# qq456cvb/CPPF

Hardware: AMD Instinct MI355X
Metric: point-pairs/sec (PPF+MLP+vote+argmax), N=4096 K=128; 1/2/4/8 GPU (higher is better)
Workload: dtype f32; 1 GPU; c2: single object N=4096 K=128 (P=524288 pairs), bottle config, res 0.004, grid 26x76x26, num_rots 72 adaptive, fused PPF+MLP(MFMA f32)+decode of the  ... (full text: bench_full.json); parallelism=objects x1

## Files before the change

### cppf_amd/csrc/pair_mlp.hip

```cpp
#include <hip/hip_runtime.h>
#include <stdint.h>
#include <string.h>

#include "../../include/cppf.h"
#include "cppf_math.h"

using namespace cppf;

typedef float f32x4 __attribute__((ext_vector_type(4)));
typedef float f32x2 __attribute__((ext_vector_type(2)));
typedef float f32x4u __attribute__((ext_vector_type(4), aligned(4)));

#define CPPF_CHECK_LAUNCH()                         \
    do {                                            \
        hipError_t e__ = hipGetLastError();         \
        if (e__ != hipSuccess) return (int)e__;     \
    } while (0)

#include "pair_layout.h"

static bool is_std(int F, const int* dims, int n_res, int out_dim)
{
    return F == STD_F && n_res == 3 && dims[0] == 84 && dims[1] == 32 && dims[2] == 32 && dims[3] == 16 &&
           out_dim >= 1 && out_dim <= 16 * STD_NOB;
}

#define GEN_MAX_RES 8
#define GEN_MAX_DIM 128
static bool gen_ok(int F, const int* dims, int n_res, int out_dim)
{
    if (n_res < 0 || n_res > GEN_MAX_RES || F < 1 || out_dim < 1 || out_dim > 1024) return false;
    if (dims[0] != 2 * F + 4) return false;
    for (int i = 0; i <= n_res; ++i)
        if (dims[i] < 1 || dims[i] > GEN_MAX_DIM) return false;
    return true;
}
static size_t gen_floats(const int* dims, int n_res, int out_dim)
{
    size_t n = 0;
    for (int i = 0; i < n_res; ++i) {
        size_t K = dims[i], M = dims[i + 1];
        n += M * K + M + M * M + M;
        if (K != M) n += M * K + M;
    }
    n += (size_t)out_dim * dims[n_res] + out_dim;
    return n;
}

extern "C" size_t cppf_pair_mlp_packed_floats(int F, const int* dims, int n_res, int out_dim)
{
    if (!dims) return 0;
    if (is_std(F, dims, n_res, out_dim)) return STD_PACKED;
    if (gen_ok(F, dims, n_res, out_dim)) return gen_floats(dims, n_res, out_dim);
    return 0;
}

extern "C" int cppf_pair_mlp_pack(const float* params, const int64_t* offs, int F, const int* dims, int n_res,
                                  int out_dim, float* out)
{
    if (!params || !offs || !dims || !out) return CPPF_EINVAL;
    if (is_std(F, dims, n_res, out_dim)) {
        if (offs[4] < 0 || offs[10] >= 0 || offs[16] < 0) return CPPF_EINVAL;
        for (int i = 0; i < STD_PACKED; ++i) out[i] = std_pack_elem(i, params, offs, out_dim);
        return 0;
    }
    if (gen_ok(F, dims, n_res, out_dim)) {
        size_t n = 0;
        for (int i = 0; i < n_res; ++i) {
            size_t K = dims[i], M = dims[i + 1];
            const int64_t* o = offs + 6 * i;
            if ((K != M) != (o[4] >= 0)) return CPPF_EINVAL;
            memcpy(out + n, params + o[0], sizeof(float) * M * K); n += M * K;
            memcpy(out + n, params + o[1], sizeof(float) * M); n += M;
            memcpy(out + n, params + o[2], sizeof(float) * M * M); n += M * M;
            memcpy(out + n, params + o[3], sizeof(float) * M); n += M;
            if (K != M) {
                memcpy(out + n, params + o[4], sizeof(float) * M * K); n += M * K;
                memcpy(out + n, params + o[5], sizeof(float) * M); n += M;
            }
        }
        const int64_t* o = offs + 6 * n_res;
        memcpy(out + n, params + o[0], sizeof(float) * out_dim * dims[n_res]); n += (size_t)out_dim * dims[n_res];
        memcpy(out + n, params + o[1], sizeof(float) * out_dim);
        return 0;
    }
    return CPPF_EUNSUPPORTED;
}

struct PackOffs { int64_t o[20]; };
__global__ __launch_bounds__(256) void pair_pack_kernel(const float* __restrict__ params, PackOffs offs, int out_dim,
                                                        float* __restrict__ out)
{
    const int i = blockIdx.x * 256 + threadIdx.x;
    if (i < STD_PACKED) out[i] = std_pack_elem(i, params, offs.o, out_dim);
}
extern "C" int cppf_pair_mlp_pack_device(const float* params, const int64_t* offs, int F, const int* dims, int n_res,
                                         int out_dim, float* out, void* stream)
{
    if (!params || !offs || !dims || !out) return CPPF_EINVAL;
    if (!is_std(F, dims, n_res, out_dim)) return CPPF_EUNSUPPORTED;
    if (offs[4] < 0 || offs[10] >= 0 || offs[16] < 0) return CPPF_EINVAL;
    PackOffs po;
    for (int i = 0; i < 20; ++i) po.o[i] = offs[i];
    hipLaunchKernelGGL(pair_pack_kernel, dim3((STD_PACKED + 255) / 256), dim3(256), 0, (hipStream_t)stream, params, po,
                       out_dim, out);
    hipError_t e = hipGetLastError();
    return e == hipSuccess ? 0 : (int)e;
}

#define MLP_THREADS 1024
#define MLP_WAVES_PER_SIMD 4
#define PB 1

__device__ __forceinline__ f32x4 mfma4(float a, float b, f32x4 c)
{
    return __builtin_amdgcn_mfma_f32_16x16x4f32(a, b, c, 0, 0, 0);
}
__device__ __forceinline__ float relu1(float v) { return fmaxf(v, 0.f); }
__device__ __forceinline__ f32x4 relu4(f32x4 v)
{
    f32x4 r;
    r[0] = relu1(v[0]); r[1] = relu1(v[1]); r[2] = relu1(v[2]); r[3] = relu1(v[3]);
    return r;
}
__device__ __forceinline__ f32x4 ldb4(const float* p) { return *reinterpret_cast<const f32x4*>(p); }

__device__ __forceinline__ float ppf_component(const float* __restrict__ pc, const float* __restrict__ nrm, int a, int b,
                                               int g)
{
    const f3 pa = ld3(pc, a), pb = ld3(pc, b), na = ld3(nrm, a), nb = ld3(nrm, b);
    const f3 xy = sub3(pa, pb);
    const float d = sqrtf((xy.x * xy.x + xy.y * xy.y) + xy.z * xy.z);
    const float den = d + 1e-7f;
    const f3 u = {xy.x / den, xy.y / den, xy.z / den};
    const float p0 = (na.x * u.x + na.y * u.y) + na.z * u.z;
    const float p1 = (nb.x * u.x + nb.y * u.y) + nb.z * u.z;
    const float p2 = (na.x * nb.x + na.y * nb.y) + na.z * nb.z;
    return g == 0 ? p0 : (g == 1 ? p1 : (g == 2 ? p2 : d));
}

__device__ __forceinline__ unsigned xor16u(unsigned v, int lane)
{
    (void)lane;
    return (unsigned)__builtin_amdgcn_ds_swizzle((int)v, 0x401f);
}
__device__ __forceinline__ unsigned xor32u(unsigned v, int lane)
{
    return (unsigned)__builtin_amdgcn_ds_bpermute((lane ^ 32) << 2, (int)v);
}
__device__ __forceinline__ float xor16f(float v, int lane) { return __uint_as_float(xor16u(__float_as_uint(v), lane)); }
__device__ __forceinline__ float xor32f(float v, int lane) { return __uint_as_float(xor32u(__float_as_uint(v), lane)); }

template <int NL>
__device__ __forceinline__ bool sample_seg(const float (&v)[NL], float u, int g, int lane, int& bin)
{
    static_assert(NL == 8 || NL == 9, "the draw below searches 7 running sums + at most one more");
    float m = v[0];
#pragma unroll
    for (int k = 1; k < NL; ++k) m = fmaxf(m, v[k]);
    float mall = fmaxf(m, xor16f(m, lane));
    mall = fmaxf(mall, xor32f(mall, lane));
    const float c = -(mall * CPPF_LOG2E);
    float e[NL];
#pragma unroll
    for (int k = 0; k < NL; ++k) e[k] = det_exp2w(v[k], c);
    float b[NL];
    b[0] = e[0];
#pragma unroll
    for (int k = 1; k < NL; ++k) b[k] = b[k - 1] + e[k];
    const float T = b[NL - 1];
    const float Tp = xor16f(T, lane);
    const float half = T + Tp;
    const float oth = xor32f(half, lane);
    const float off = ((g & 2) ? oth : 0.f) + ((g & 1) ? Tp : 0.f);
    const float t = u * ((g & 2) ? oth + half : half + oth) - off;
    const bool c1 = b[3] > t;
    const bool c2 = (c1 ? b[1] : b[5]) > t;
    const float lo = c2 ? b[0] : b[2], hi = c2 ? b[4] : b[6];
    const bool c3 = (c1 ? lo : hi) > t;
    int kk = (c1 ? 0 : 4) + (c2 ? 0 : 2) + (c3 ? 0 : 1);
    if (NL == 9) kk = b[7] > t ? kk : 8;
    const unsigned long long hm = __ballot(b[NL - 1] > t);
    const unsigned h0 = (unsigned)hm & 0xffffu, h1 = (unsigned)(hm >> 16) & 0xffffu, h2 = (unsigned)(hm >> 32) & 0xffffu;
    const unsigned o1 = h1 & ~h0, o2 = h2 & ~(h0 | h1), o3 = ~(h0 | h1 | h2) & 0xffffu;
    const unsigned long long own = (unsigned long long)(h0 | (o1 << 16)) | ((unsigned long long)(o2 | (o3 << 16)) << 32);
    bool owner = __builtin_amdgcn_inverse_ballot_w64(own);
    bin = NL * g + kk;
    if (__any(u < 0.f)) {
        asm volatile("" ::: "memory");
        int ak = 64;
#pragma unroll
        for (int k = NL - 1; k >= 0; --k)
            if (v[k] == mall) ak = k;
        const int am = NL * g + ak;
        int best = min(am, (int)xor16u((unsigned)am, lane));
        best = min(best, (int)xor32u((unsigned)best, lane));
        if (u < 0.f) { bin = best; owner = am == best; }
    }
    return owner;
}

struct MlpArgs {
    const float* pc;
    const float* nrm;
    const float* feat;
    const void* idxs;
    const float* packed;
    const float* u_tr;
    const float* u_rot;
    const float* table;
    float* out;
    float* outputs;
    float* heads;
    int64_t P;
    int out_dim;
    int idx64;
    float vr0, vr1;
    const int32_t* sel;
    const int32_t* n_sel;
};

template <typename T>
__device__ __forceinline__ const T& at_off(const void* base, unsigned byte_off)
{
    return *reinterpret_cast<const T*>(static_cast<const char*>(base) + byte_off);
}
template <typename T>
__device__ __forceinline__ T& at_off(void* base, unsigned byte_off)
{
    return *reinterpret_cast<T*>(static_cast<char*>(base) + byte_off);
}
__device__ __forceinline__ f3 ld3o(const float* __restrict__ base, int i)
{
    const unsigned o = __umul24((unsigned)i, 12u);
    return {at_off<float>(base, o), at_off<float>(base + 1, o), at_off<float>(base + 2, o)};
}

template <bool SEL>
__device__ __forceinline__ unsigned pair_row(const MlpArgs& A, int slot, int Pn)
{
    const unsigned s = (unsigned)min(slot, Pn - 1);
    return SEL ? (unsigned)at_off<int>(A.sel, s * 4u) : s;
}

template <bool SEL>
__device__ __forceinline__ void load_pair_idx(const MlpArgs& A, int slot, int Pn, int& ia, int& ib)
{
    const unsigned p = pair_row<SEL>(A, slot, Pn);
    const unsigned o = p * (A.idx64 ? 16u : 8u);
    ia = at_off<int>(A.idxs, o);
    ib = at_off<int>(static_cast<const char*>(A.idxs) + (A.idx64 ? 8 : 4), o);
}

__device__ __forceinline__ float ppf_from(f3 pa, f3 pb, f3 na, f3 nb, int g)
{
    const f3 xy = sub3(pa, pb);
    const float d = sqrt_rn((xy.x * xy.x + xy.y * xy.y) + xy.z * xy.z);
    const float den = d + 1e-7f;
    const float rden = refined_rcp(den);
    const f3 u = {div_by(xy.x, den, rden), div_by(xy.y, den, rden), div_by(xy.z, den, rden)};
    const float p0 = (na.x * u.x + na.y * u.y) + na.z * u.z;
    const float p1 = (nb.x * u.x + nb.y * u.y) + nb.z * u.z;
    const float p2 = (na.x * nb.x + na.y * nb.y) + na.z * nb.z;
    (void)g;
    const bool g0 = __builtin_amdgcn_inverse_ballot_w64(0x000000000000ffffull), g1 = __builtin_amdgcn_inverse_ballot_w64(0x00000000ffff0000ull),
               g2 = __builtin_amdgcn_inverse_ballot_w64(0x0000ffff00000000ull);
    const float s23 = g2 ? p2 : d, s123 = g1 ? p1 : s23;
    return g0 ? p0 : s123;
}

#define PROJ_PPB 8
__device__ __forceinline__ void point_proj_body(const float* __restrict__ feat, const float* __restrict__ packed, float* __restrict__ T,
                                                int64_t N)
{
    __shared__ float f[PROJ_PPB][STD_F];
    const int half = threadIdx.x >> 7, r = threadIdx.x & 127;
    const int64_t n0 = (int64_t)blockIdx.x * PROJ_PPB;
    for (int i = threadIdx.x; i < PROJ_PPB * STD_F; i += 256) {
        const int64_t n = n0 + i / STD_F;
        f[i / STD_F][i % STD_F] = n < N ? feat[n * STD_F + i % STD_F] : 0.f;
    }
    __syncthreads();
    float acc[PROJ_PPB / 2];
    const float b = r < 64 ? packed[OFF_BPT + r] : 0.f;
#pragma unroll
    for (int q = 0; q < PROJ_PPB / 2; ++q) acc[q] = b;
#pragma unroll 8
    for (int k = 0; k < STD_F; ++k) {
        const float w = packed[OFF_WPT + k * PROJ_COLS + r];
#pragma unroll
        for (int q = 0; q < PROJ_PPB / 2; ++q) acc[q] = fmaf(w, f[half + 2 * q][k], acc[q]);
    }
#pragma unroll
    for (int q = 0; q < PROJ_PPB / 2; ++q) {
        const int64_t n = n0 + half + 2 * q;
        if (n < N) T[n * PROJ_COLS + r] = acc[q];
    }
}
__global__ __launch_bounds__(256) void point_proj_kernel(const float* __restrict__ feat, const float* __restrict__ packed,
                                                         float* __restrict__ T, int64_t N)
{
    point_proj_body(feat, packed, T, N);
}
struct ProjBatch { const float* feat[8]; const float* packed[8]; float* table[8]; int64_t N[8]; };
__global__ __launch_bounds__(256) void point_proj_batch_kernel(ProjBatch B)
{
    const int i = blockIdx.y;
    if ((int64_t)blockIdx.x * PROJ_PPB >= B.N[i]) return;
    point_proj_body(B.feat[i], B.packed[i], B.table[i], B.N[i]);
}

template <bool LOGITS, bool DECODE, bool HEADS, bool SEL>
__device__ __forceinline__ void pair_mlp_body(const MlpArgs& A, const int wg, const int n_wg)
{
    extern __shared__ __attribute__((aligned(16))) float W[];
    {
        const f32x4* src = reinterpret_cast<const f32x4*>(A.packed);
        f32x4* dst = reinterpret_cast<f32x4*>(W);
        for (int k = threadIdx.x; k < STD_LDS / 4; k += MLP_THREADS) {
            int from = k;
            if (DECODE && k >= OFF_WF / 4 && k < OFF_B0B / 4) from = OFF_WFD / 4 + (k - OFF_WF / 4);
            if (DECODE && k >= OFF_BF / 4) from = OFF_BFD / 4 + (k - OFF_BF / 4);
            dst[k] = src[from];
        }
    }
    float* lut = W + STD_LDS;
    int* tile_ctr = reinterpret_cast<int*>(W + STD_LDS + 112);
    if (threadIdx.x == 0) *tile_ctr = 0;
    if (DECODE && threadIdx.x < 100) {
        const int k = threadIdx.x;
        float v;
        if (k < 32) v = ((float)k / 31.0f * 2.0f) * A.vr0 - A.vr0;
        else if (k < 64) v = (float)(k - 32) / 31.0f * A.vr1;
        else v = (float)(k - 64) / 35.0f * (float)CPPF_PI;
        lut[k] = v;
    }
    __syncthreads();

    const int lane = threadIdx.x & 63;
    const int j = lane & 15, g = lane >> 4;
    __builtin_assume(g >= 0 && g < 4);
    int Pn = (int)A.P;
    if (SEL) Pn = min(max(*A.n_sel, 0), Pn);
    const int n_tiles = (Pn + 16 * PB - 1) / (16 * PB);
    const int per_wg = (n_tiles + n_wg - 1) / n_wg;
    const int wg_begin = wg * per_wg;
    const int wg_end = min(wg_begin + per_wg, n_tiles);
    auto claim = [&]() -> int {
        int v = 0;
        if (lane == 0) v = atomicAdd(tile_ctr, 1);
        return wg_begin + __builtin_amdgcn_readfirstlane(v);
    };
    int cur = claim();
    if (cur >= wg_end) return;
    int nxt = claim();

    f32x4 acc[PB][4];
    int ia1[PB], ib1[PB];
    {
        f32x4 ta[PB][4], tb[PB][4];
        float xp[PB];
        int ia[PB], ib[PB];
#pragma unroll
        for (int pb = 0; pb < PB; ++pb) load_pair_idx<SEL>(A, cur * (16 * PB) + pb * 16 + j, Pn, ia[pb], ib[pb]);
#pragma unroll
        for (int pb = 0; pb < PB; ++pb) {
            const unsigned oa = (unsigned)ia[pb] * (PROJ_COLS * 4u) + 16u * g, ob_ = (unsigned)ib[pb] * (PROJ_COLS * 4u) + 256u + 16u * g;
#pragma unroll
            for (int ob = 0; ob < 4; ++ob) { ta[pb][ob] = at_off<f32x4>(A.table, oa + 64u * ob); tb[pb][ob] = at_off<f32x4>(A.table, ob_ + 64u * ob); }
            xp[pb] = ppf_from(ld3o(A.pc, ia[pb]), ld3o(A.pc, ib[pb]), ld3o(A.nrm, ia[pb]), ld3o(A.nrm, ib[pb]), g);
        }
        const int nt = nxt < wg_end ? nxt : cur;
#pragma unroll
        for (int pb = 0; pb < PB; ++pb) load_pair_idx<SEL>(A, nt * (16 * PB) + pb * 16 + j, Pn, ia1[pb], ib1[pb]);
        const f32x4 w = ldb4(W + OFF_W0P + lane * 4);
#pragma unroll
        for (int ob = 0; ob < 4; ++ob)
#pragma unroll
            for (int pb = 0; pb < PB; ++pb) acc[pb][ob] = mfma4(w[ob], xp[pb], ta[pb][ob] + tb[pb][ob]);
    }

    for (;;) {
        const int tile = cur;
        asm volatile("" ::: "memory");
        int pair[PB];
#pragma unroll
        for (int pb = 0; pb < PB; ++pb) pair[pb] = tile * (16 * PB) + pb * 16 + j;
        unsigned row[PB];
#pragma unroll
        for (int pb = 0; pb < PB; ++pb) row[pb] = pair_row<SEL>(A, pair[pb], Pn);

        f3 npa[PB], npb[PB], nna[PB], nnb[PB];
#pragma unroll
        for (int pb = 0; pb < PB; ++pb) {
            npa[pb] = ld3o(A.pc, ia1[pb]); npb[pb] = ld3o(A.pc, ib1[pb]);
            nna[pb] = ld3o(A.nrm, ia1[pb]); nnb[pb] = ld3o(A.nrm, ib1[pb]);
        }
        f32x2 ut[PB], ur[PB];
        if (DECODE) {
#pragma unroll
            for (int pb = 0; pb < PB; ++pb) {
                const unsigned po = row[pb] * 8u;
                if (!SEL) ut[pb] = at_off<f32x2>(A.u_tr, po);
                if (HEADS) ur[pb] = at_off<f32x2>(A.u_rot, po);
            }
        }

        f32x4 y[PB][2];
        {
            f32x4 h[PB][2], a2[PB][2];
#pragma unroll
            for (int pb = 0; pb < PB; ++pb) { h[pb][0] = relu4(acc[pb][0]); h[pb][1] = relu4(acc[pb][1]); }
#pragma unroll
            for (int ob = 0; ob < 2; ++ob) {
                const f32x4 b = ldb4(W + OFF_B0B + 16 * ob + 4 * g);
#pragma unroll
                for (int pb = 0; pb < PB; ++pb) a2[pb][ob] = b;
            }
#pragma unroll
            for (int s = 0; s < 8; ++s) {
                const f32x2 w = *reinterpret_cast<const f32x2*>(W + OFF_W0B + (s * 64 + lane) * 2);
#pragma unroll
                for (int ob = 0; ob < 2; ++ob)
#pragma unroll
                    for (int pb = 0; pb < PB; ++pb) a2[pb][ob] = mfma4(w[ob], h[pb][s >> 2][s & 3], a2[pb][ob]);
            }
#pragma unroll
            for (int pb = 0; pb < PB; ++pb) { y[pb][0] = a2[pb][0] + acc[pb][2]; y[pb][1] = a2[pb][1] + acc[pb][3]; }
        }
        {
            f32x4 a1[PB][2], h[PB][2], a2[PB][2];
#pragma unroll
            for (int ob = 0; ob < 2; ++ob) {
                const f32x4 b1 = ldb4(W + OFF_B1A + 16 * ob + 4 * g), b2 = ldb4(W + OFF_B1B + 16 * ob + 4 * g);
#pragma unroll
                for (int pb = 0; pb < PB; ++pb) { a1[pb][ob] = b1; a2[pb][ob] = b2; }
            }
#pragma unroll
            for (int s = 0; s < 8; ++s) {
                const f32x2 w = *reinterpret_cast<const f32x2*>(W + OFF_W1A + (s * 64 + lane) * 2);
#pragma unroll
                for (int ob = 0; ob < 2; ++ob)
#pragma unroll
                    for (int pb = 0; pb < PB; ++pb) a1[pb][ob] = mfma4(w[ob], y[pb][s >> 2][s & 3], a1[pb][ob]);
            }
#pragma unroll
            for (int pb = 0; pb < PB; ++pb) { h[pb][0] = relu4(a1[pb][0]); h[pb][1] = relu4(a1[pb][1]); }
#pragma unroll
            for (int s = 0; s < 8; ++s) {
                const f32x2 w = *reinterpret_cast<const f32x2*>(W + OFF_W1B + (s * 64 + lane) * 2);
#pragma unroll
                for (int ob = 0; ob < 2; ++ob)
#pragma unroll
                    for (int pb = 0; pb < PB; ++pb) a2[pb][ob] = mfma4(w[ob], h[pb][s >> 2][s & 3], a2[pb][ob]);
            }
#pragma unroll
            for (int pb = 0; pb < PB; ++pb) { y[pb][0] = a2[pb][0] + y[pb][0]; y[pb][1] = a2[pb][1] + y[pb][1]; }
        }
        f32x4 ta[PB][4], tb[PB][4];
        float xp[PB];
#pragma unroll
        for (int pb = 0; pb < PB; ++pb) {
            xp[pb] = ppf_from(npa[pb], npb[pb], nna[pb], nnb[pb], g);
            const unsigned oa = (unsigned)ia1[pb] * (PROJ_COLS * 4u) + 16u * g, ob_ = (unsigned)ib1[pb] * (PROJ_COLS * 4u) + 256u + 16u * g;
#pragma unroll
            for (int ob = 0; ob < 4; ++ob) { ta[pb][ob] = at_off<f32x4>(A.table, oa + 64u * ob); tb[pb][ob] = at_off<f32x4>(A.table, ob_ + 64u * ob); }
        }
        const int nxt2 = claim();
        {
            const int nt = nxt2 < wg_end ? nxt2 : tile;
#pragma unroll
            for (int pb = 0; pb < PB; ++pb) load_pair_idx<SEL>(A, nt * (16 * PB) + pb * 16 + j, Pn, ia1[pb], ib1[pb]);
        }

        f32x4 z[PB];
        {
            f32x4 a1[PB][2], a2[PB];
            {
                const f32x4 b1 = ldb4(W + OFF_B2 + 4 * g), b0 = ldb4(W + OFF_B2 + 16 + 4 * g), b2 = ldb4(W + OFF_B2B + 4 * g);
#pragma unroll
                for (int pb = 0; pb < PB; ++pb) { a1[pb][0] = b1; a1[pb][1] = b0; a2[pb] = b2; }
            }
#pragma unroll
            for (int s = 0; s < 8; ++s) {
                const f32x2 w = *reinterpret_cast<const f32x2*>(W + OFF_W2 + (s * 64 + lane) * 2);
#pragma unroll
                for (int ob = 0; ob < 2; ++ob)
#pragma unroll
                    for (int pb = 0; pb < PB; ++pb) a1[pb][ob] = mfma4(w[ob], y[pb][s >> 2][s & 3], a1[pb][ob]);
            }
#pragma unroll
            for (int s = 0; s < 4; ++s) {
                const float w = W[OFF_W2B + s * 64 + lane];
#pragma unroll
                for (int pb = 0; pb < PB; ++pb) {
                    const f32x4 h = relu4(a1[pb][0]);
                    a2[pb] = mfma4(w, h[s], a2[pb]);
                }
            }
#pragma unroll
            for (int pb = 0; pb < PB; ++pb) z[pb] = a2[pb] + a1[pb][1];
        }
        {
            const f32x4 w = ldb4(W + OFF_W0P + lane * 4);
#pragma unroll
            for (int ob = 0; ob < 4; ++ob)
#pragma unroll
                for (int pb = 0; pb < PB; ++pb) acc[pb][ob] = mfma4(w[ob], xp[pb], ta[pb][ob] + tb[pb][ob]);
        }
#pragma unroll
        for (int pb = 0; pb < PB; ++pb) {
            constexpr int NOB_USED = (DECODE && !HEADS) ? 4 : STD_NOB;
            f32x4 L[STD_NOB];
#pragma unroll
            for (int ob = 0; ob < NOB_USED; ++ob) L[ob] = ldb4(W + OFF_BF + 16 * ob + 4 * g);
#pragma unroll
            for (int s = 0; s < 4; ++s) {
                const float* wp = W + OFF_WF + (s * 64 + lane) * STD_NOBP;
                const f32x4 w0 = ldb4(wp), w1 = ldb4(wp + 4), w2 = ldb4(wp + 8);
#pragma unroll
                for (int ob = 0; ob < NOB_USED; ++ob) {
                    const float w = ob < 4 ? w0[ob & 3] : (ob < 8 ? w1[ob & 3] : w2[ob & 3]);
                    L[ob] = mfma4(w, z[pb][s], L[ob]);
                }
            }
            const bool live = pair[pb] < Pn;
            if (!LOGITS && !DECODE) {
                float sacc = 0.f;
#pragma unroll
                for (int ob = 0; ob < STD_NOB; ++ob) sacc += (L[ob][0] + L[ob][1]) + (L[ob][2] + L[ob][3]);
                if (sacc == 1.2345e30f) A.outputs[0] = sacc;
            }
            if (LOGITS) {
                if (live) {
                    float* o = A.out + (int64_t)pair[pb] * A.out_dim + 4 * g;
#pragma unroll
                    for (int ob = 0; ob < STD_NOB; ++ob) {
                        const int c0 = 16 * ob + 4 * g;
                        if (c0 + 3 < A.out_dim) {
                            *reinterpret_cast<f32x4u*>(o + 16 * ob) = L[ob];
                        } else {
#pragma unroll
                            for (int r = 0; r < 3; ++r)
                                if (c0 + r < A.out_dim) o[16 * ob + r] = L[ob][r];
                        }
                    }
                }
            }
            if (DECODE) {
                int k;
                if (!SEL) {
                    {
                        const float v[8] = {L[0][0], L[0][1], L[0][2], L[0][3], L[1][0], L[1][1], L[1][2], L[1][3]};
                        if (sample_seg<8>(v, ut[pb][0], g, lane, k) && live) at_off<float>(A.outputs, row[pb] * 8u) = lut[k];
                    }
                    {
                        const float v[8] = {L[2][0], L[2][1], L[2][2], L[2][3], L[3][0], L[3][1], L[3][2], L[3][3]};
                        if (sample_seg<8>(v, ut[pb][1], g, lane, k) && live) at_off<float>(A.outputs, row[pb] * 8u + 4u) = lut[32 + k];
                    }
                }
                if (HEADS) {
                    const unsigned ho = row[pb] * 32u;
                    {
                        const float v[9] = {L[4][0], L[4][1], L[4][2], L[4][3], L[5][0], L[5][1], L[5][2], L[5][3], L[8][0]};
                        if (sample_seg<9>(v, ur[pb][0], g, lane, k) && live) at_off<float>(A.heads, ho) = lut[64 + k];
                    }
                    {
                        const float v[9] = {L[6][0], L[6][1], L[6][2], L[6][3], L[7][0], L[7][1], L[7][2], L[7][3], L[8][1]};
                        if (sample_seg<9>(v, ur[pb][1], g, lane, k) && live) at_off<float>(A.heads, ho + 4u) = lut[64 + k];
                    }
                    if (live && g < 2) { f32x2 w; w[0] = L[8][2]; w[1] = L[8][3]; at_off<f32x2>(A.heads, ho + 8u + 8u * g) = w; }
                    if (live && g == 2) { f32x2 w; w[0] = L[8][2]; w[1] = 0.f; at_off<f32x2>(A.heads, ho + 24u) = w; }
                }
            }
        }
        cur = nxt;
        nxt = nxt2;
        if (cur >= wg_end) break;
    }
}

template <bool LOGITS, bool DECODE, bool HEADS, bool SEL = false>
__global__ __launch_bounds__(MLP_THREADS, MLP_WAVES_PER_SIMD) void pair_mlp_kernel(MlpArgs A)
{
    pair_mlp_body<LOGITS, DECODE, HEADS, SEL>(A, (int)blockIdx.x, (int)gridDim.x);
}

#define MLP_BATCH_MAX 8
struct MlpBatch {
    MlpArgs item[MLP_BATCH_MAX];
    int wg_begin[MLP_BATCH_MAX + 1];
    int n;
    int per_xcd;
};
static_assert(sizeof(ProjBatch) <= 4096, "ProjBatch travels by value: kernel arguments are limited to 4 KB");
static_assert(sizeof(MlpBatch) <= 4096, "MlpBatch travels by value: kernel arguments are limited to 4 KB");
template <bool HEADS, bool SEL = false>
__global__ __launch_bounds__(MLP_THREADS, MLP_WAVES_PER_SIMD) void pair_mlp_batch_kernel(MlpBatch B)
{
    if (!SEL && B.per_xcd > 0) {
        const int x = (int)blockIdx.x & 7, r = (int)blockIdx.x >> 3;
        const int i = x / B.per_xcd;
        pair_mlp_body<false, true, HEADS, false>(B.item[i], r * B.per_xcd + x % B.per_xcd, ((int)gridDim.x >> 3) * B.per_xcd);
        return;
    }
    int i = 0;
    while (i + 1 < B.n && (int)blockIdx.x >= B.wg_begin[i + 1]) ++i;
    pair_mlp_body<false, true, HEADS, SEL>(B.item[i], (int)blockIdx.x - B.wg_begin[i], B.wg_begin[i + 1] - B.wg_begin[i]);
}

struct GenArgs {
    const float* pc;
    const float* nrm;
    const float* feat;
    const void* idxs;
    const float* packed;
    float* out;
    int64_t P;
    int F, n_res, out_dim, idx64;
    int dims[GEN_MAX_RES + 1];
};
#define GEN_THREADS 64
__global__ __launch_bounds__(GEN_THREADS) void pair_mlp_generic_kernel(GenArgs A)
{
    extern __shared__ __attribute__((aligned(16))) float S[];
    int maxd = 0;
    for (int i = 0; i <= A.n_res; ++i) maxd = max(maxd, A.dims[i]);
    float* X = S;
    float* H = S + maxd * GEN_THREADS;
    const int t = threadIdx.x;
    for (int64_t p = (int64_t)blockIdx.x * GEN_THREADS + t; p < (A.P + GEN_THREADS - 1) / GEN_THREADS * GEN_THREADS;
         p += (int64_t)gridDim.x * GEN_THREADS) {
        const bool live = p < A.P;
        const int64_t pc_ = live ? p : A.P - 1;
        int ia, ib;
        if (A.idx64) {
            const longlong2 v = reinterpret_cast<const longlong2*>(A.idxs)[pc_];
            ia = (int)v.x; ib = (int)v.y;
        } else {
            const int2 v = reinterpret_cast<const int2*>(A.idxs)[pc_];
            ia = v.x; ib = v.y;
        }
        const int F = A.F;
        for (int k = 0; k < F; ++k) {
            X[k * GEN_THREADS + t] = A.feat[(int64_t)ia * F + k];
            X[(F + k) * GEN_THREADS + t] = A.feat[(int64_t)ib * F + k];
        }
        for (int c = 0; c < 4; ++c) X[(2 * F + c) * GEN_THREADS + t] = ppf_component(A.pc, A.nrm, ia, ib, c);
        const float* w = A.packed;
        for (int l = 0; l < A.n_res; ++l) {
            const int K = A.dims[l], M = A.dims[l + 1];
            const float *w1 = w, *b1 = w1 + M * K, *w2 = b1 + M, *b2 = w2 + M * M;
            const float *w0 = b2 + M, *b0 = w0 + M * K;
            const bool has0 = K != M;
            for (int o = 0; o < M; ++o) {
                float acc = b1[o];
                for (int k = 0; k < K; ++k) acc = fmaf(w1[o * K + k], X[k * GEN_THREADS + t], acc);
                H[o * GEN_THREADS + t] = acc > 0.f ? acc : 0.f;
            }
            for (int o = 0; o < M; ++o) {
                float acc = b2[o];
                for (int k = 0; k < M; ++k) acc = fmaf(w2[o * M + k], H[k * GEN_THREADS + t], acc);
                float skip;
                if (has0) {
                    float a0 = b0[o];
                    for (int k = 0; k < K; ++k) a0 = fmaf(w0[o * K + k], X[k * GEN_THREADS + t], a0);
                    skip = a0;
                } else {
                    skip = X[o * GEN_THREADS + t];
                }
                S[(2 * maxd + o) * GEN_THREADS + t] = acc + skip;
            }
            for (int o = 0; o < M; ++o) X[o * GEN_THREADS + t] = S[(2 * maxd + o) * GEN_THREADS + t];
            w = has0 ? b0 + M : b2 + M;
        }
        const int K = A.dims[A.n_res];
        const float *wf = w, *bf = wf + A.out_dim * K;
        for (int o = 0; o < A.out_dim; ++o) {
            float acc = bf[o];
            for (int k = 0; k < K; ++k) acc = fmaf(wf[o * K + k], X[k * GEN_THREADS + t], acc);
            if (live) A.out[p * A.out_dim + o] = acc;
        }
    }
}

__device__ int sample_bin_mem(const float* __restrict__ l, int nb, float u, int col0)
{
    (void)col0;
    float m = l[0];
    int am = 0;
    for (int k = 1; k < nb; ++k)
        if (l[k] > m) { m = l[k]; am = k; }
    if (u < 0.f) return am;
    const int NL = (nb + 3) / 4;
    const float c = -(m * CPPF_LOG2E);
    float T[4];
    for (int g = 0; g < 4; ++g) {
        float acc = 0.f;
        for (int k = g * NL; k < (g + 1) * NL && k < nb; ++k) {
            const float ek = det_exp2w(l[k], c);
            acc = k == g * NL ? ek : acc + ek;
        }
        T[g] = acc;
    }
    const float s01 = T[0] + T[1], s23 = T[2] + T[3];
    const float tt = u * (s01 + s23);
    const float off[4] = {0.f, T[0], s01, s01 + T[2]};
    for (int g = 0; g < 4; ++g) {
        const float t = tt - off[g];
        float b = 0.f;
        for (int k = g * NL; k < (g + 1) * NL && k < nb; ++k) {
            const float ek = det_exp2w(l[k], c);
            b = k == g * NL ? ek : b + ek;
            if (b > t) return k;
        }
    }
    return nb - 1;
}


__global__ __launch_bounds__(256) void decode_center_kernel(const float* __restrict__ logits, int64_t P, int ld, int nb,
                                                            float vr0, float vr1, const float* __restrict__ u,
                                                            float* __restrict__ outputs)
{
    const int64_t i = (int64_t)blockIdx.x * 256 + threadIdx.x;
    if (i >= 2 * P) return;
    const int64_t p = i >> 1;
    const int h = (int)(i & 1);
    const int k = sample_bin_mem(logits + p * ld + h * nb, nb, u[i], h * nb);
    const float d = (float)(nb - 1);
    outputs[i] = h == 0 ? ((float)k / d * 2.0f) * vr0 - vr0 : (float)k / d * vr1;
}

__global__ __launch_bounds__(256) void decode_rot_kernel(const float* __restrict__ logits, int64_t P, int ld, int out_dim,
                                                         int tb, int rb, const float* __restrict__ u,
                                                         float* __restrict__ heads)
{
    const int64_t i = (int64_t)blockIdx.x * 256 + threadIdx.x;
    if (i >= 2 * P) return;
    const int64_t p = i >> 1;
    const int h = (int)(i & 1);
    const float* l = logits + p * ld;
    const int k = sample_bin_mem(l + 2 * tb + h * rb, rb, u[i], 2 * tb + h * rb);
    float* o = heads + 8 * p;
    o[h] = (float)k / (float)(rb - 1) * (float)CPPF_PI;
    if (h == 0) { o[2] = l[out_dim - 5]; o[3] = l[out_dim - 4]; o[4] = l[out_dim - 3]; }
    else { o[5] = l[out_dim - 2]; o[6] = l[out_dim - 1]; o[7] = 0.f; }
}

static int mlp_grid(int64_t P)
{
    const int64_t tiles = (P + 16 * PB - 1) / (16 * PB);
    int64_t nb = (tiles + MLP_THREADS / 64 - 1) / (MLP_THREADS / 64);
    const int64_t resident = 256 * (MLP_WAVES_PER_SIMD * 4 / (MLP_THREADS / 64));
    if (nb > resident) nb = resident;
    if (nb < 1) nb = 1;
    return (int)nb;
}

extern "C" size_t cppf_pair_mlp_workspace_bytes(int64_t N, int F, const int* dims, int n_res, int out_dim)
{
    if (!dims || N < 0) return 0;
    return is_std(F, dims, n_res, out_dim) ? (size_t)N * PROJ_COLS * sizeof(float) : 0;
}

template <bool LOGITS, bool DECODE, bool HEADS, bool SEL = false>
static int launch_std(MlpArgs& A, int64_t N, void* workspace, size_t workspace_bytes, hipStream_t st)
{
    if (N < 1) return CPPF_EINVAL;
    if (N >= (1ll << 23) || A.P >= (1ll << 27)) return CPPF_EUNSUPPORTED;
    if (!workspace || workspace_bytes < (size_t)N * PROJ_COLS * sizeof(float)) return CPPF_EWORKSPACE;
    float* table = static_cast<float*>(workspace);
    if (!SEL) {
        hipLaunchKernelGGL(point_proj_kernel, dim3((unsigned)((N + PROJ_PPB - 1) / PROJ_PPB)), dim3(256), 0, st, A.feat, A.packed, table, N);
        CPPF_CHECK_LAUNCH();
    }
    A.table = table;
    static bool attr_done = false;
    if (!attr_done) {
        hipError_t e = hipFuncSetAttribute(reinterpret_cast<const void*>(&pair_mlp_kernel<LOGITS, DECODE, HEADS, SEL>),
                                           hipFuncAttributeMaxDynamicSharedMemorySize, (STD_LDS + 128) * sizeof(float));
        if (e != hipSuccess) return (int)e;
        attr_done = true;
    }
    hipLaunchKernelGGL((pair_mlp_kernel<LOGITS, DECODE, HEADS, SEL>), dim3(mlp_grid(A.P)), dim3(MLP_THREADS),
                       (STD_LDS + 128) * sizeof(float), st, A);
    CPPF_CHECK_LAUNCH();
    return 0;
}

extern "C" int cppf_pair_mlp_forward(const float* pc, const float* nrm, const float* feat, const void* idxs,
                                     int idx_is_i64, const float* packed, int64_t N, int F, const int* dims, int n_res,
                                     int64_t P, int out_dim, float* out, void* workspace, size_t workspace_bytes,
                                     void* stream)
{
    if (P < 0 || !dims) return CPPF_EINVAL;
    if (P == 0) return 0;
    if (!pc || !nrm || !feat || !idxs || !packed || !out) return CPPF_EINVAL;
    hipStream_t st = (hipStream_t)stream;
    if (is_std(F, dims, n_res, out_dim)) {
        MlpArgs A = {};
        A.pc = pc; A.nrm = nrm; A.feat = feat; A.idxs = idxs; A.packed = packed; A.out = out; A.P = P;
        A.out_dim = out_dim; A.idx64 = idx_is_i64;
        return launch_std<true, false, false>(A, N, workspace, workspace_bytes, st);
    }
    if (!gen_ok(F, dims, n_res, out_dim)) return CPPF_EUNSUPPORTED;
    GenArgs G = {};
    G.pc = pc; G.nrm = nrm; G.feat = feat; G.idxs = idxs; G.packed = packed; G.out = out; G.P = P;
    G.F = F; G.n_res = n_res; G.out_dim = out_dim; G.idx64 = idx_is_i64;
    int maxd = 0;
    for (int i = 0; i <= n_res; ++i) { G.dims[i] = dims[i]; if (dims[i] > maxd) maxd = dims[i]; }
    const size_t lds = (size_t)3 * maxd * GEN_THREADS * sizeof(float);
    static bool attr_done = false;
    if (!attr_done) {
        (void)hipFuncSetAttribute(reinterpret_cast<const void*>(&pair_mlp_generic_kernel),
                            hipFuncAttributeMaxDynamicSharedMemorySize, 3 * GEN_MAX_DIM * GEN_THREADS * sizeof(float));
        attr_done = true;
    }
    int64_t nb = (P + GEN_THREADS - 1) / GEN_THREADS;
    if (nb > 4096) nb = 4096;
    hipLaunchKernelGGL(pair_mlp_generic_kernel, dim3((unsigned)nb), dim3(GEN_THREADS), lds, st, G);
    CPPF_CHECK_LAUNCH();
    return 0;
}

extern "C" int cppf_pair_mlp_decode(const float* pc, const float* nrm, const float* feat, const void* idxs,
                                    int idx_is_i64, const float* packed, int64_t N, int F, const int* dims, int n_res,
                                    int64_t P, int out_dim, int tr_bins, int rot_bins, float vr0, float vr1,
                                    const float* u_tr, const float* u_rot, float* outputs, float* heads,
                                    void* workspace, size_t workspace_bytes, void* stream)
{
    if (P < 0 || !dims) return CPPF_EINVAL;
    if (!is_std(F, dims, n_res, out_dim) || tr_bins != 32 || rot_bins != 36 || out_dim != 141) return CPPF_EUNSUPPORTED;
    if (P == 0) return 0;
    if (!pc || !nrm || !feat || !idxs || !packed || !u_tr || !outputs) return CPPF_EINVAL;
    if ((heads != nullptr) != (u_rot != nullptr)) return CPPF_EINVAL;
    MlpArgs A = {};
    A.pc = pc; A.nrm = nrm; A.feat = feat; A.idxs = idxs; A.packed = packed; A.P = P; A.out_dim = out_dim;
    A.idx64 = idx_is_i64; A.u_tr = u_tr; A.u_rot = u_rot; A.outputs = outputs; A.heads = heads; A.vr0 = vr0; A.vr1 = vr1;
    return heads ? launch_std<false, true, true>(A, N, workspace, workspace_bytes, (hipStream_t)stream)
                 : launch_std<false, true, false>(A, N, workspace, workspace_bytes, (hipStream_t)stream);
}

static void batch_plan(int n_items, const int64_t* n_pairs, int* wg_begin, int* per_xcd, int* grid)
{
    int64_t tiles_all = 0, tmin = INT64_MAX, tmax = 0;
    for (int i = 0; i < n_items; ++i) {
        const int64_t tiles = (n_pairs[i] + 15) / 16;
        tiles_all += tiles;
        tmin = tiles < tmin ? tiles : tmin; tmax = tiles > tmax ? tiles : tmax;
    }
    const int total = mlp_grid(tiles_all * 16) < n_items ? n_items : mlp_grid(tiles_all * 16);
    int given = 0;
    for (int i = 0; i < n_items; ++i) {
        const int64_t tiles = (n_pairs[i] + 15) / 16;
        int w = (int)((tiles * total + tiles_all - 1) / tiles_all);
        const int left = total - given - (n_items - 1 - i);
        if (w > left) w = left;
        if (w < 1) w = 1;
        wg_begin[i] = given;
        given += w;
    }
    wg_begin[n_items] = given;
    *per_xcd = 0;
    if (8 % n_items == 0 && tmax * 10 <= tmin * 11 && given >= 8) {
        *per_xcd = 8 / n_items;
        given = given / 8 * 8;
    }
    *grid = given;
}

extern "C" int cppf_pair_mlp_batch_plan(int n_items, const int64_t* n_pairs, int* per_xcd, int* grid, int* wg_begin)
{
    if (n_items < 1 || n_items > MLP_BATCH_MAX || !n_pairs || !per_xcd || !grid) return CPPF_EINVAL;
    for (int i = 0; i < n_items; ++i)
        if (n_pairs[i] < 1 || n_pairs[i] >= (1ll << 27)) return CPPF_EINVAL;
    int wb[MLP_BATCH_MAX + 1];
    batch_plan(n_items, n_pairs, wb, per_xcd, grid);
    if (wg_begin)
        for (int i = 0; i <= n_items; ++i) wg_begin[i] = wb[i];
    return 0;
}

extern "C" int cppf_pair_mlp_decode_batch(int n_items, const CppfPairMlpItem* items, int F, const int* dims, int n_res, int out_dim,
                                          int tr_bins, int rot_bins, void* stream)
{
    if (n_items < 1 || n_items > MLP_BATCH_MAX || !items || !dims) return CPPF_EINVAL;
    if (!is_std(F, dims, n_res, out_dim) || tr_bins != 32 || rot_bins != 36 || out_dim != 141) return CPPF_EUNSUPPORTED;
    hipStream_t st = (hipStream_t)stream;
    MlpBatch B = {};
    B.n = n_items;
    const bool heads = items[0].heads != nullptr;
    int64_t n_pairs[MLP_BATCH_MAX];
    int given = 0;
    for (int i = 0; i < n_items; ++i) {
        const CppfPairMlpItem& it = items[i];
        n_pairs[i] = it.n_pairs;
        if (it.n_pairs < 1 || it.n_points < 1) return CPPF_EINVAL;
        if (!it.pc || !it.nrm || !it.feat || !it.idxs || !it.packed || !it.u_tr || !it.outputs) return CPPF_EINVAL;
        if ((it.heads != nullptr) != heads || (it.heads != nullptr) != (it.u_rot != nullptr)) return CPPF_EINVAL;
        if (it.n_points >= (1ll << 23) || it.n_pairs >= (1ll << 27)) return CPPF_EUNSUPPORTED;
        if (!it.workspace || it.workspace_bytes < (size_t)it.n_points * PROJ_COLS * sizeof(float)) return CPPF_EWORKSPACE;
    }
    batch_plan(n_items, n_pairs, B.wg_begin, &B.per_xcd, &given);
    ProjBatch PJ = {};
    int64_t proj_blocks = 1;
    for (int i = 0; i < n_items; ++i) {
        const CppfPairMlpItem& it = items[i];
        float* table = static_cast<float*>(it.workspace);
        PJ.feat[i] = it.feat; PJ.packed[i] = it.packed; PJ.table[i] = table; PJ.N[i] = it.n_points;
        const int64_t nb = (it.n_points + PROJ_PPB - 1) / PROJ_PPB;
        proj_blocks = nb > proj_blocks ? nb : proj_blocks;
        MlpArgs& A = B.item[i];
        A.pc = it.pc; A.nrm = it.nrm; A.feat = it.feat; A.idxs = it.idxs; A.packed = it.packed; A.P = it.n_pairs; A.out_dim = out_dim;
        A.idx64 = it.idx_is_i64; A.u_tr = it.u_tr; A.u_rot = it.u_rot; A.outputs = it.outputs; A.heads = it.heads;
        A.vr0 = it.vr0; A.vr1 = it.vr1; A.table = table;
    }
    hipLaunchKernelGGL(point_proj_batch_kernel, dim3((unsigned)proj_blocks, (unsigned)n_items), dim3(256), 0, st, PJ);
    CPPF_CHECK_LAUNCH();
    static bool attr_done[2] = {false, false};
    const void* fn = heads ? reinterpret_cast<const void*>(&pair_mlp_batch_kernel<true>) : reinterpret_cast<const void*>(&pair_mlp_batch_kernel<false>);
    if (!attr_done[heads]) {
        hipError_t e = hipFuncSetAttribute(fn, hipFuncAttributeMaxDynamicSharedMemorySize, (STD_LDS + 128) * sizeof(float));
        if (e != hipSuccess) return (int)e;
        attr_done[heads] = true;
    }
    if (heads) hipLaunchKernelGGL((pair_mlp_batch_kernel<true>), dim3((unsigned)given), dim3(MLP_THREADS), (STD_LDS + 128) * sizeof(float), st, B);
    else hipLaunchKernelGGL((pair_mlp_batch_kernel<false>), dim3((unsigned)given), dim3(MLP_THREADS), (STD_LDS + 128) * sizeof(float), st, B);
    CPPF_CHECK_LAUNCH();
    return 0;
}

extern "C" int cppf_pair_mlp_decode_sel_batch(int n_items, const CppfPairMlpItem* items, int F, const int* dims, int n_res, int out_dim,
                                              int tr_bins, int rot_bins, void* stream)
{
    if (n_items < 1 || n_items > MLP_BATCH_MAX || !items || !dims) return CPPF_EINVAL;
    if (!is_std(F, dims, n_res, out_dim) || tr_bins != 32 || rot_bins != 36 || out_dim != 141) return CPPF_EUNSUPPORTED;
    MlpBatch B = {};
    int given = 0;
    for (int i = 0; i < n_items; ++i) {
        const CppfPairMlpItem& it = items[i];
        if (it.n_pairs < 0 || it.max_sel < 0) return CPPF_EINVAL;
        if (it.n_pairs == 0 || it.max_sel == 0) continue;
        if (it.n_pairs >= (1ll << 27) || it.n_points >= (1ll << 23)) return CPPF_EUNSUPPORTED;
        if (!it.pc || !it.nrm || !it.feat || !it.idxs || !it.packed || !it.u_rot || !it.sel || !it.n_sel_dev || !it.heads) return CPPF_EINVAL;
        if (!it.workspace || it.workspace_bytes < (size_t)it.n_points * PROJ_COLS * sizeof(float)) return CPPF_EWORKSPACE;
        MlpArgs& A = B.item[B.n];
        A.pc = it.pc; A.nrm = it.nrm; A.feat = it.feat; A.idxs = it.idxs; A.packed = it.packed; A.out_dim = out_dim;
        A.P = it.max_sel < it.n_pairs ? it.max_sel : it.n_pairs;
        A.idx64 = it.idx_is_i64; A.u_rot = it.u_rot; A.heads = it.heads; A.sel = it.sel; A.n_sel = it.n_sel_dev;
        A.table = static_cast<const float*>(it.workspace);
        B.wg_begin[B.n] = given;
        int w = mlp_grid(A.P);
        const int cap = mlp_grid(1ll << 26) / (n_items > 1 ? 2 : 1);
        if (w > cap) w = cap;
        given += w;
        ++B.n;
    }
    if (B.n == 0) return 0;
    B.wg_begin[B.n] = given;
    static bool attr_done = false;
    const void* fn = reinterpret_cast<const void*>(&pair_mlp_batch_kernel<true, true>);
    if (!attr_done) {
        hipError_t e = hipFuncSetAttribute(fn, hipFuncAttributeMaxDynamicSharedMemorySize, (STD_LDS + 128) * sizeof(float));
        if (e != hipSuccess) return (int)e;
        attr_done = true;
    }
    hipLaunchKernelGGL((pair_mlp_batch_kernel<true, true>), dim3((unsigned)given), dim3(MLP_THREADS), (STD_LDS + 128) * sizeof(float),
                       (hipStream_t)stream, B);
    CPPF_CHECK_LAUNCH();
    return 0;
}

extern "C" int cppf_pair_mlp_decode_sel(const float* pc, const float* nrm, const float* feat, const void* idxs,
                                        int idx_is_i64, const float* packed, int64_t N, int F, const int* dims, int n_res,
                                        int64_t P, int out_dim, int tr_bins, int rot_bins, const float* u_rot,
                                        const int32_t* sel, const int32_t* n_sel_dev, int64_t max_sel, float* heads,
                                        void* workspace, size_t workspace_bytes, void* stream)
{
    if (P < 0 || max_sel < 0 || !dims) return CPPF_EINVAL;
    if (!is_std(F, dims, n_res, out_dim) || tr_bins != 32 || rot_bins != 36 || out_dim != 141) return CPPF_EUNSUPPORTED;
    if (P == 0 || max_sel == 0) return 0;
    if (P >= (1ll << 27)) return CPPF_EUNSUPPORTED;
    if (!pc || !nrm || !feat || !idxs || !packed || !u_rot || !sel || !n_sel_dev || !heads) return CPPF_EINVAL;
    MlpArgs A = {};
    A.pc = pc; A.nrm = nrm; A.feat = feat; A.idxs = idxs; A.packed = packed; A.out_dim = out_dim;
    A.P = max_sel < P ? max_sel : P;
    A.idx64 = idx_is_i64; A.u_rot = u_rot; A.heads = heads; A.sel = sel; A.n_sel = n_sel_dev;
    return launch_std<false, true, true, true>(A, N, workspace, workspace_bytes, (hipStream_t)stream);
}

#ifdef CPPF_DEBUG_ENTRY
extern "C" int cppf_debug_mlp_chain_only(const float* pc, const float* nrm, const float* feat, const void* idxs,
                                         int idx_is_i64, const float* packed, int64_t N, int64_t P, float* scratch,
                                         void* workspace, size_t workspace_bytes, void* stream)
{
    if (!pc || !nrm || !feat || !idxs || !packed || !scratch || P < 1) return CPPF_EINVAL;
    MlpArgs A = {};
    A.pc = pc; A.nrm = nrm; A.feat = feat; A.idxs = idxs; A.packed = packed; A.P = P; A.out_dim = 141;
    A.idx64 = idx_is_i64; A.outputs = scratch;
    return launch_std<false, false, false>(A, N, workspace, workspace_bytes, (hipStream_t)stream);
}
#endif

extern "C" int cppf_decode_center(const float* logits, int64_t P, int ld, int tr_bins, float vr0, float vr1,
                                  const float* u_tr, float* outputs, void* stream)
{
    if (P < 0 || tr_bins < 2 || ld < 2 * tr_bins) return CPPF_EINVAL;
    if (P == 0) return 0;
    if (!logits || !u_tr || !outputs) return CPPF_EINVAL;
    hipLaunchKernelGGL(decode_center_kernel, dim3((unsigned)((2 * P + 255) / 256)), dim3(256), 0, (hipStream_t)stream,
                       logits, P, ld, tr_bins, vr0, vr1, u_tr, outputs);
    CPPF_CHECK_LAUNCH();
    return 0;
}

extern "C" int cppf_decode_rot(const float* logits, int64_t P, int ld, int out_dim, int tr_bins, int rot_bins,
                               const float* u_rot, float* heads, void* stream)
{
    if (P < 0 || rot_bins < 2 || out_dim < 2 * tr_bins + 2 * rot_bins + 5 || ld < out_dim) return CPPF_EINVAL;
    if (P == 0) return 0;
    if (!logits || !u_rot || !heads) return CPPF_EINVAL;
    hipLaunchKernelGGL(decode_rot_kernel, dim3((unsigned)((2 * P + 255) / 256)), dim3(256), 0, (hipStream_t)stream,
                       logits, P, ld, out_dim, tr_bins, rot_bins, u_rot, heads);
    CPPF_CHECK_LAUNCH();
    return 0;
}
```

Measured before the change: 6.602 billion pairs/s.

## Process pair tiles in runs of four with lane-shuffled PPF and index handout

Each wave now claims four 16-pair tiles at once and loads indices and computes PPF features for all 64 pairs one per lane, then hands the per-tile values to the MFMA lane layout with ds_bpermute. This replaces four redundant per-tile PPF computations (each done by 4 lane groups) and cuts atomic claims by four. It adds bpermute traffic per tile, coarser work claiming that can worsen load balance at tail, and restructures the batch kernel dispatch into a single body call. In the non-SEL path the branch now also passes SEL as its template argument, which is false there, so that path's behaviour is unchanged.

```diff
diff --git a/cppf_amd/csrc/pair_mlp.hip b/cppf_amd/csrc/pair_mlp.hip
--- a/cppf_amd/csrc/pair_mlp.hip
+++ b/cppf_amd/csrc/pair_mlp.hip
@@ -111,6 +111,8 @@
 #define MLP_THREADS 1024
 #define MLP_WAVES_PER_SIMD 4
 #define PB 1
+#define MLP_RUN 4
+static_assert(PB == 1 && 16 * PB * MLP_RUN == 64, "a run is the 64 pairs a wave holds one per lane");
 
 __device__ __forceinline__ f32x4 mfma4(float a, float b, f32x4 c)
 {
@@ -243,16 +245,20 @@
     return SEL ? (unsigned)at_off<int>(A.sel, s * 4u) : s;
 }
 
+struct RunIdx { int ia, ib; unsigned row; };
 template <bool SEL>
-__device__ __forceinline__ void load_pair_idx(const MlpArgs& A, int slot, int Pn, int& ia, int& ib)
-{
-    const unsigned p = pair_row<SEL>(A, slot, Pn);
-    const unsigned o = p * (A.idx64 ? 16u : 8u);
-    ia = at_off<int>(A.idxs, o);
-    ib = at_off<int>(static_cast<const char*>(A.idxs) + (A.idx64 ? 8 : 4), o);
-}
-
-__device__ __forceinline__ float ppf_from(f3 pa, f3 pb, f3 na, f3 nb, int g)
+__device__ __forceinline__ RunIdx load_run_idx(const MlpArgs& A, int slot, int Pn)
+{
+    RunIdx r;
+    r.row = pair_row<SEL>(A, slot, Pn);
+    const unsigned o = r.row * (A.idx64 ? 16u : 8u);
+    r.ia = at_off<int>(A.idxs, o);
+    r.ib = at_off<int>(static_cast<const char*>(A.idxs) + (A.idx64 ? 8 : 4), o);
+    return r;
+}
+
+struct Ppf { float p0, p1, p2, d; };
+__device__ __forceinline__ Ppf ppf_from(f3 pa, f3 pb, f3 na, f3 nb)
 {
     const f3 xy = sub3(pa, pb);
     const float d = sqrt_rn((xy.x * xy.x + xy.y * xy.y) + xy.z * xy.z);
@@ -262,7 +268,14 @@
     const float p0 = (na.x * u.x + na.y * u.y) + na.z * u.z;
     const float p1 = (nb.x * u.x + nb.y * u.y) + nb.z * u.z;
     const float p2 = (na.x * nb.x + na.y * nb.y) + na.z * nb.z;
-    (void)g;
+    return {p0, p1, p2, d};
+}
+
+__device__ __forceinline__ int from_lane(unsigned src, int v) { return __builtin_amdgcn_ds_bpermute((int)src, v); }
+__device__ __forceinline__ float from_lane(unsigned src, float v) { return __int_as_float(__builtin_amdgcn_ds_bpermute((int)src, __float_as_int(v))); }
+__device__ __forceinline__ float ppf_hand_out(unsigned src, const Ppf& x)
+{
+    const float p0 = from_lane(src, x.p0), p1 = from_lane(src, x.p1), p2 = from_lane(src, x.p2), d = from_lane(src, x.d);
     const bool g0 = __builtin_amdgcn_inverse_ballot_w64(0x000000000000ffffull), g1 = __builtin_amdgcn_inverse_ballot_w64(0x00000000ffff0000ull),
                g2 = __builtin_amdgcn_inverse_ballot_w64(0x0000ffff00000000ull);
     const float s23 = g2 ? p2 : d, s123 = g1 ? p1 : s23;
@@ -348,53 +361,47 @@
     const int wg_end = min(wg_begin + per_wg, n_tiles);
     auto claim = [&]() -> int {
         int v = 0;
-        if (lane == 0) v = atomicAdd(tile_ctr, 1);
+        if (lane == 0) v = atomicAdd(tile_ctr, MLP_RUN);
         return wg_begin + __builtin_amdgcn_readfirstlane(v);
     };
     int cur = claim();
     if (cur >= wg_end) return;
     int nxt = claim();
 
+    RunIdx ri = load_run_idx<SEL>(A, cur * 16 + lane, Pn);
+    Ppf rx = ppf_from(ld3o(A.pc, ri.ia), ld3o(A.pc, ri.ib), ld3o(A.nrm, ri.ia), ld3o(A.nrm, ri.ib));
+    RunIdx ni;
+    unsigned row_n = 0;
     f32x4 acc[PB][4];
-    int ia1[PB], ib1[PB];
     {
-        f32x4 ta[PB][4], tb[PB][4];
-        float xp[PB];
-        int ia[PB], ib[PB];
-#pragma unroll
-        for (int pb = 0; pb < PB; ++pb) load_pair_idx<SEL>(A, cur * (16 * PB) + pb * 16 + j, Pn, ia[pb], ib[pb]);
-#pragma unroll
-        for (int pb = 0; pb < PB; ++pb) {
-            const unsigned oa = (unsigned)ia[pb] * (PROJ_COLS * 4u) + 16u * g, ob_ = (unsigned)ib[pb] * (PROJ_COLS * 4u) + 256u + 16u * g;
-#pragma unroll
-            for (int ob = 0; ob < 4; ++ob) { ta[pb][ob] = at_off<f32x4>(A.table, oa + 64u * ob); tb[pb][ob] = at_off<f32x4>(A.table, ob_ + 64u * ob); }
-            xp[pb] = ppf_from(ld3o(A.pc, ia[pb]), ld3o(A.pc, ib[pb]), ld3o(A.nrm, ia[pb]), ld3o(A.nrm, ib[pb]), g);
-        }
+        f32x4 ta[4], tb[4];
+        const unsigned src = 4u * j;
+        const int ia = from_lane(src, ri.ia), ib = from_lane(src, ri.ib);
+        if (SEL) row_n = (unsigned)from_lane(src, (int)ri.row);
+        const unsigned oa = (unsigned)ia * (PROJ_COLS * 4u) + 16u * g, ob_ = (unsigned)ib * (PROJ_COLS * 4u) + 256u + 16u * g;
+#pragma unroll
+        for (int ob = 0; ob < 4; ++ob) { ta[ob] = at_off<f32x4>(A.table, oa + 64u * ob); tb[ob] = at_off<f32x4>(A.table, ob_ + 64u * ob); }
+        const float xp = ppf_hand_out(src, rx);
         const int nt = nxt < wg_end ? nxt : cur;
-#pragma unroll
-        for (int pb = 0; pb < PB; ++pb) load_pair_idx<SEL>(A, nt * (16 * PB) + pb * 16 + j, Pn, ia1[pb], ib1[pb]);
+        ni = load_run_idx<SEL>(A, nt * 16 + lane, Pn);
         const f32x4 w = ldb4(W + OFF_W0P + lane * 4);
 #pragma unroll
-        for (int ob = 0; ob < 4; ++ob)
-#pragma unroll
-            for (int pb = 0; pb < PB; ++pb) acc[pb][ob] = mfma4(w[ob], xp[pb], ta[pb][ob] + tb[pb][ob]);
-    }
-
+        for (int ob = 0; ob < 4; ++ob) acc[0][ob] = mfma4(w[ob], xp, ta[ob] + tb[ob]);
+    }
+
+    int q = 0, nq = min(MLP_RUN, wg_end - cur);
     for (;;) {
-        const int tile = cur;
         asm volatile("" ::: "memory");
         int pair[PB];
-#pragma unroll
-        for (int pb = 0; pb < PB; ++pb) pair[pb] = tile * (16 * PB) + pb * 16 + j;
+        pair[0] = (cur + q) * 16 + j;
         unsigned row[PB];
-#pragma unroll
-        for (int pb = 0; pb < PB; ++pb) row[pb] = pair_row<SEL>(A, pair[pb], Pn);
+        row[0] = SEL ? row_n : (unsigned)min(pair[0], Pn - 1);
+        const bool last = q + 1 == nq;
 
         f3 npa[PB], npb[PB], nna[PB], nnb[PB];
-#pragma unroll
-        for (int pb = 0; pb < PB; ++pb) {
-            npa[pb] = ld3o(A.pc, ia1[pb]); npb[pb] = ld3o(A.pc, ib1[pb]);
-            nna[pb] = ld3o(A.nrm, ia1[pb]); nnb[pb] = ld3o(A.nrm, ib1[pb]);
+        if (last) {
+            npa[0] = ld3o(A.pc, ni.ia); npb[0] = ld3o(A.pc, ni.ib);
+            nna[0] = ld3o(A.nrm, ni.ia); nnb[0] = ld3o(A.nrm, ni.ib);
         }
         f32x2 ut[PB], ur[PB];
         if (DECODE) {
@@ -457,20 +464,24 @@
 #pragma unroll
             for (int pb = 0; pb < PB; ++pb) { y[pb][0] = a2[pb][0] + y[pb][0]; y[pb][1] = a2[pb][1] + y[pb][1]; }
         }
+        if (last) {
+            ri = ni;
+            rx = ppf_from(npa[0], npb[0], nna[0], nnb[0]);
+            cur = nxt;
+            nxt = claim();
+            const int nt = nxt < wg_end ? nxt : cur;
+            ni = load_run_idx<SEL>(A, nt * 16 + lane, Pn);
+        }
+        const unsigned src = 4u * j + 64u * (last ? 0 : q + 1);
         f32x4 ta[PB][4], tb[PB][4];
         float xp[PB];
-#pragma unroll
-        for (int pb = 0; pb < PB; ++pb) {
-            xp[pb] = ppf_from(npa[pb], npb[pb], nna[pb], nnb[pb], g);
-            const unsigned oa = (unsigned)ia1[pb] * (PROJ_COLS * 4u) + 16u * g, ob_ = (unsigned)ib1[pb] * (PROJ_COLS * 4u) + 256u + 16u * g;
-#pragma unroll
-            for (int ob = 0; ob < 4; ++ob) { ta[pb][ob] = at_off<f32x4>(A.table, oa + 64u * ob); tb[pb][ob] = at_off<f32x4>(A.table, ob_ + 64u * ob); }
-        }
-        const int nxt2 = claim();
         {
-            const int nt = nxt2 < wg_end ? nxt2 : tile;
-#pragma unroll
-            for (int pb = 0; pb < PB; ++pb) load_pair_idx<SEL>(A, nt * (16 * PB) + pb * 16 + j, Pn, ia1[pb], ib1[pb]);
+            const int ia = from_lane(src, ri.ia), ib = from_lane(src, ri.ib);
+            if (SEL) row_n = (unsigned)from_lane(src, (int)ri.row);
+            xp[0] = ppf_hand_out(src, rx);
+            const unsigned oa = (unsigned)ia * (PROJ_COLS * 4u) + 16u * g, ob_ = (unsigned)ib * (PROJ_COLS * 4u) + 256u + 16u * g;
+#pragma unroll
+            for (int ob = 0; ob < 4; ++ob) { ta[0][ob] = at_off<f32x4>(A.table, oa + 64u * ob); tb[0][ob] = at_off<f32x4>(A.table, ob_ + 64u * ob); }
         }
 
         f32x4 z[PB];
@@ -574,9 +585,13 @@
                 }
             }
         }
-        cur = nxt;
-        nxt = nxt2;
-        if (cur >= wg_end) break;
+        if (last) {
+            if (cur >= wg_end) break;
+            q = 0;
+            nq = min(MLP_RUN, wg_end - cur);
+        } else {
+            ++q;
+        }
     }
 }
 
@@ -598,15 +613,18 @@
 template <bool HEADS, bool SEL = false>
 __global__ __launch_bounds__(MLP_THREADS, MLP_WAVES_PER_SIMD) void pair_mlp_batch_kernel(MlpBatch B)
 {
+    int i = 0, wg, n_wg;
     if (!SEL && B.per_xcd > 0) {
         const int x = (int)blockIdx.x & 7, r = (int)blockIdx.x >> 3;
-        const int i = x / B.per_xcd;
-        pair_mlp_body<false, true, HEADS, false>(B.item[i], r * B.per_xcd + x % B.per_xcd, ((int)gridDim.x >> 3) * B.per_xcd);
-        return;
-    }
-    int i = 0;
-    while (i + 1 < B.n && (int)blockIdx.x >= B.wg_begin[i + 1]) ++i;
-    pair_mlp_body<false, true, HEADS, SEL>(B.item[i], (int)blockIdx.x - B.wg_begin[i], B.wg_begin[i + 1] - B.wg_begin[i]);
+        i = x / B.per_xcd;
+        wg = r * B.per_xcd + x % B.per_xcd;
+        n_wg = ((int)gridDim.x >> 3) * B.per_xcd;
+    } else {
+        while (i + 1 < B.n && (int)blockIdx.x >= B.wg_begin[i + 1]) ++i;
+        wg = (int)blockIdx.x - B.wg_begin[i];
+        n_wg = B.wg_begin[i + 1] - B.wg_begin[i];
+    }
+    pair_mlp_body<false, true, HEADS, SEL>(B.item[i], wg, n_wg);
 }
 
 struct GenArgs {
```

New measurement: 6.511 billion pairs/s. 0.986x the previous value.
